# fab-jul/L3C-PyTorch

Hardware: AMD Instinct MI355X
Metric: MPix/s encode (net+CDF+AC) on 768x512 RGB (higher is better)
Workload: dtype f32; 1 GPU; L3C 0306_0001 (cr.cf, synthetic seeded checkpoint), batch of 768x512 synthetic RGB per GPU: net forward + fused logistic-mixture CDF head + HIP range coder -> bytes in HBM; checkpoint=calibrated, batch_per_gpu=128, image=768x512, coder_cus=0

## Files before the change

l3c-pytorch_amd/_lib.py:

```python
import ctypes
import os

import torch

_HERE = os.path.dirname(os.path.abspath(__file__))
LIB_PATH = os.environ.get('L3C_LIB') or os.path.join(_HERE, 'csrc', 'libl3c_hip.so')

c_i64, c_int, c_vp, c_f32 = ctypes.c_int64, ctypes.c_int, ctypes.c_void_p, ctypes.c_float


class L3CError(RuntimeError):
    pass


class ConvDesc(ctypes.Structure):
    _fields_ = [('inp', c_vp), ('in_cstride', c_int), ('in_coff', c_int),
                ('packed_w', c_vp), ('bias', c_vp),
                ('residual', c_vp), ('res_cstride', c_int), ('res_coff', c_int),
                ('out', c_vp), ('out_cstride', c_int), ('out_coff', c_int),
                ('B', c_int), ('Hin', c_int), ('Win', c_int), ('Cin', c_int), ('Cout', c_int),
                ('KS', c_int), ('stride', c_int), ('dilation', c_int), ('epilogue', c_int)]


class AcGroup(ctypes.Structure):
# ... 195 lines not shown
XCHECK_PROTOTYPES = {
    'l3c_conv_wino_packed_words': (c_i64, [c_int, c_int]),
    'l3c_conv_wino_pack_weights': (c_int, [c_vp, c_int, c_int, c_vp, c_vp]),
    'l3c_conv_wino': (c_int, [ctypes.POINTER(ConvDesc), c_vp]),
    'l3c_conv_wino_set_tiles_per_block': (c_int, [c_int]),
    'l3c_xcheck_sigmoid_exhaustive': (c_int, [c_vp, c_vp, c_vp]),
    'l3c_conv_wino4w_packed_words': (c_i64, [c_int, c_int]),
    'l3c_conv_wino4w_pack_weights': (c_int, [c_vp, c_int, c_int, c_vp, c_vp]),
    'l3c_conv_wino4w': (c_int, [ctypes.POINTER(ConvDesc), c_int, c_vp]),
}
XCHECK_SMALL_PROTOTYPES = {
    'l3c_xcheck_rgb_head': (c_int, [c_vp, c_vp, c_vp, c_vp, c_vp, c_vp, c_vp, c_int, c_int, c_int, c_int, c_vp, c_vp, c_vp]),
    'l3c_xcheck_to_q_quantize': (c_int, [c_vp, c_vp, c_vp, c_vp, c_i64, c_i64, c_int, c_int, c_int, c_vp, c_vp, c_vp, c_vp]),
    'l3c_xcheck_dec_head': (c_int, [c_vp, c_vp, c_vp, c_vp, c_i64, c_i64, c_int, c_int, c_vp, c_vp]),
}
XCHECK_LIB_PATH = os.environ.get('L3C_XCHECK_LIB') or os.path.join(_HERE, 'csrc', 'libl3c_hip_xcheck.so')

_lib = None
_xcheck = None


def load():
    global _lib
    if _lib is None:
        _snapshot_queues()
        if not os.path.isfile(LIB_PATH):
            raise L3CError('libl3c_hip.so not found at {} -- build it with `python l3c-pytorch_amd/csrc/build.py` '
                           '(or __graft_entry__.build()); there is no CPU fallback.'.format(LIB_PATH))
        lib = ctypes.CDLL(LIB_PATH)
        for name, (res, args) in PROTOTYPES.items():
            fn = getattr(lib, name)
            fn.restype, fn.argtypes = res, args
        if lib.l3c_abi_version() != ABI_VERSION:
            raise L3CError('ABI version mismatch: library {} != binding {}'.format(lib.l3c_abi_version(), ABI_VERSION))
        _lib = lib
    return _lib


def load_xcheck():
    global _xcheck
    if _xcheck is None:
        if not os.path.isfile(XCHECK_LIB_PATH):
            raise L3CError('libl3c_hip_xcheck.so not found at {} -- build it with `python l3c-pytorch_amd/csrc/build.py`'.format(XCHECK_LIB_PATH))
        lib = ctypes.CDLL(XCHECK_LIB_PATH)
        lib.l3c_last_error.restype = ctypes.c_char_p
        for name, (res, args) in list(XCHECK_PROTOTYPES.items()) + list(XCHECK_SMALL_PROTOTYPES.items()):
            fn = getattr(lib, name)
            fn.restype, fn.argtypes = res, args
        _xcheck = lib
    return _xcheck


def call_xcheck(name, *args):
    rc = getattr(load_xcheck(), name)(*args)
    if rc != 0:
        raise L3CError('libl3c_hip_xcheck: {} (status {})'.format(load_xcheck().l3c_last_error().decode(), rc))


def check(rc):
    if rc != 0:
        raise L3CError('libl3c_hip: {} (status {})'.format(load().l3c_last_error().decode(), rc))
# ... 60 lines not shown
```

l3c-pytorch_amd/csrc/ac_kernels.hip:

```cpp
#include <vector>

#include "ac_core.h"
#include "dmll_core.h"
#include "l3c_common.h"

namespace {

constexpr int kChunk = 64;

__device__ __forceinline__ int64_t iv_index(int64_t chunk, int64_t n_streams, int64_t s, int role, int j) {
    return ((chunk * n_streams + s) * 2 + role) * kChunk + j;
}

__global__ __launch_bounds__(256) void intervals_from_table_kernel(const uint16_t *__restrict__ cdf, int64_t row_stride,
                                                                   int Lp, const int16_t *__restrict__ sym,
                                                                   int64_t n_streams, int64_t n_sym,
                                                                   uint32_t *__restrict__ iv) {
    const int64_t n_chunks = (n_sym + kChunk - 1) / kChunk;
    const int64_t total = n_chunks * n_streams * kChunk;
    for (int64_t i = (int64_t)blockIdx.x * blockDim.x + threadIdx.x; i < total; i += (int64_t)gridDim.x * blockDim.x) {
        const int j = (int)(i % kChunk);
        const int64_t s = (i / kChunk) % n_streams;
        const int64_t chunk = i / kChunk / n_streams;
        const int64_t t = chunk * kChunk + j;
// ... 661 lines not shown

__device__ __forceinline__ Regs<4> window_full_row(const WindowCtx &w, int64_t b, int64_t n, int lane) {
    const int C = w.C, K = w.K, c = w.c;
    const float *px = w.P + (b * w.HW + n) * (int64_t)(4 * C * K);
    auto get = [&](int ch) { return px[ch]; };
    float x0 = 0.f, x1 = 0.f;
    if (c > 0) {
        x0 = (float)w.sym[(b * C + 0) * w.HW + n];
        if (c > 1) x1 = (float)w.sym[(b * C + 1) * w.HW + n];
    }
    const l3c::MixStats st = l3c::mix_stats(get, C, K, c);
    const float t0 = w.targets[lane], t1 = w.targets[lane + 64], t2 = w.targets[lane + 128], t3 = w.targets[lane + 192];
    float a0 = 0.0f, a1 = 0.0f, a2 = 0.0f, a3 = 0.0f;
    for (int k = 0; k < K; ++k) {
        const l3c::MixComponent m = l3c::mix_component(get, st, C, K, 1, c, k, x0, x1);
        const float inv = expf(-m.log_sigma);
        a0 = a0 + l3c::cdf_term(m.pi, m.mu, inv, t0);
        a1 = a1 + l3c::cdf_term(m.pi, m.mu, inv, t1);
        a2 = a2 + l3c::cdf_term(m.pi, m.mu, inv, t2);
        a3 = a3 + l3c::cdf_term(m.pi, m.mu, inv, t3);
    }
    const float scale = (float)(65536 - 256);
    return Regs<4>{l3c::cdf_quantise(a0, scale, lane), l3c::cdf_quantise(a1, scale, lane + 64), l3c::cdf_quantise(a2, scale, lane + 128),
                   l3c::cdf_quantise(a3, scale, lane + 192)};
}

__device__ __forceinline__ bool full_row_monotone(const Regs<4> &r, int lane) {
    const uint32_t na = (uint32_t)__shfl_down((int)r.a, 1, 64), nb = (uint32_t)__shfl_down((int)r.b, 1, 64);
    const uint32_t nc = (uint32_t)__shfl_down((int)r.c, 1, 64), nd = (uint32_t)__shfl_down((int)r.d, 1, 64);
    bool bad = lane < 63 && (!(r.a < na) || !(r.b < nb) || !(r.c < nc) || !(r.d < nd));
    const uint32_t b0 = lane_read(r.b, 0), c0 = lane_read(r.c, 0), d0 = lane_read(r.d, 0);
// ... 290 lines not shown
    }
}
struct LaneMixture {
    float pi, mu, inv;
};
__device__ __forceinline__ LaneMixture window_lane_mixture(const WindowCtx &w, int64_t b, int64_t n, int lane) {
    const int C = w.C, K = w.K, c = w.c;
    const float *px = w.P + (b * w.HW + n) * (int64_t)(4 * C * K);
    auto get = [&](int ch) { return px[ch]; };
    float x0 = 0.f, x1 = 0.f;
    if (c > 0) {
        x0 = (float)w.sym[(b * C + 0) * w.HW + n];
        if (c > 1) x1 = (float)w.sym[(b * C + 1) * w.HW + n];
    }
    const int k = lane < K ? lane : K - 1;
    l3c::MixStats st;
    st.max_logit = get(c * K);
    for (int j = 1; j < K; ++j) st.max_logit = fmaxf(st.max_logit, get(c * K + j));
    const float e_k = expf(get(c * K + k) - st.max_logit);
    st.denom = 0.0f;
    for (int j = 0; j < K; ++j) st.denom = st.denom + __builtin_bit_cast(float, __builtin_amdgcn_readlane(__builtin_bit_cast(int, e_k), j));
    const l3c::MixComponent m = l3c::mix_component_e(get, st, e_k, C, K, 1, c, k, x0, x1);
    return LaneMixture{m.pi, m.mu, expf(-m.log_sigma)};
}
__device__ __forceinline__ RowHi<1> window_row_at(const WindowCtx &w, const LaneMixture &mx, int wbase, int lane, bool &monotone) {
    const float t = w.targets[wbase + lane];
    float acc = 0.0f;
    for (int j = 0; j < w.K; ++j) {
        const float pi = __builtin_bit_cast(float, __builtin_amdgcn_readlane(__builtin_bit_cast(int, mx.pi), j));
        const float mu = __builtin_bit_cast(float, __builtin_amdgcn_readlane(__builtin_bit_cast(int, mx.mu), j));
        const float inv = __builtin_bit_cast(float, __builtin_amdgcn_readlane(__builtin_bit_cast(int, mx.inv), j));
        acc = acc + l3c::cdf_term(pi, mu, inv, t);
    }
    const uint32_t v = l3c::cdf_quantise(acc, (float)(65536 - 256), wbase + lane);
    const uint32_t nxt = (uint32_t)__shfl_down((int)v, 1, 64);
    monotone = !__any(lane < 63 && !(v < nxt));
    return RowHi<1>{v << 16};
}
// ... 815 lines not shown
```

l3c-pytorch_amd/csrc/build.py:

```python
import os
import subprocess
import sys

HERE = os.path.dirname(os.path.abspath(__file__))
SOURCES = ['l3c_api.hip', 'ac_kernels.hip', 'dmll_kernels.hip', 'conv_mfma.hip', 'conv_small.hip', 'container.hip', 'conv_pw.hip', 'conv_wino4.hip', 'decode_pipeline.hip',
           'net.hip', 'codec.hip']
XCHECK_SOURCES = ['l3c_api.hip', 'conv_wino.hip', 'xcheck_dmll.hip', 'conv_wino4w.hip', 'xcheck_small.hip']
HEADERS = ['ac_core.h', 'dmll_core.h', 'l3c_common.h', 'codec_plan.h', 'codec_plan_banded.h', os.path.join('..', '..', 'include', 'l3c_hip.h'), os.path.join('..', '..', 'include', 'l3c_xcheck.h'),
           os.path.join('..', '..', 'include', 'l3c_xcheck_small.h')]
LIB = os.path.join(HERE, 'libl3c_hip.so')
XCHECK_LIB = os.path.join(HERE, 'libl3c_hip_xcheck.so')
FLAGS = ['--offload-arch=gfx950', '-O3', '-std=c++17', '-fPIC', '-ffp-contract=off', '-Wall', '-Wno-unused-function']
SOURCE_FLAGS = {'conv_wino.hip': ['-fno-slp-vectorize'], 'conv_pw.hip': ['-fno-slp-vectorize'], 'conv_wino4.hip': ['-fno-slp-vectorize'],
                'conv_wino4w.hip': ['-fno-slp-vectorize']}


def _stale(target, deps):
    if not os.path.isfile(target):
        return True
    t = os.path.getmtime(target)
    return any(os.path.getmtime(d) > t for d in deps)


def build(force=False, verbose=False, extra=(), lib=LIB, objdir='_obj', xcheck=True):
# ... 47 lines not shown
```

l3c-pytorch_amd/csrc/dmll_core.h:

```cpp
#ifndef L3C_DMLL_CORE_H_
#define L3C_DMLL_CORE_H_

#include <hip/hip_runtime.h>

namespace l3c {

__device__ __forceinline__ float sigmoid_f(float a) { return 1.0f / (1.0f + expf(-a)); }

__device__ __forceinline__ float sigmoid_mid(float a) {
    const float kNegLog2e = __uint_as_float(0xbfb8aa3bu);
    const float kNegLog2eLo = __uint_as_float(0xb2a5705fu);
    const float t = kNegLog2e * a;
    const float n = __builtin_rintf(t);
    float f = t - n;
    float c = __builtin_fmaf(a, kNegLog2e, -t);
    c = __builtin_fmaf(kNegLog2eLo, a, c);
    f = f + c;
    const float e = __builtin_amdgcn_ldexpf(__builtin_amdgcn_exp2f(f), (int)n);
    const float d = 1.0f + e;
    float r = __builtin_amdgcn_rcpf(d);
    r = __builtin_fmaf(__builtin_fmaf(-d, r, 1.0f), r, r);
    float q = r;
    q = __builtin_fmaf(__builtin_fmaf(-d, q, 1.0f), r, q);
    return __builtin_fmaf(__builtin_fmaf(-d, q, 1.0f), r, q);
}

__device__ __forceinline__ float sigmoid_sat(float a) {
    if (a >= 16.7f) return 1.0f;
    if (a <= -89.0f) return 0.0f;
    if (a > -80.0f) return sigmoid_mid(a);
    return sigmoid_f(a);
}

constexpr float kLogScalesMin = -7.0f;

struct MixStats {
    float max_logit, denom;
};

template <class Get>
__device__ __forceinline__ MixStats mix_stats(Get get, int C, int K, int c) {
    MixStats s;
    s.max_logit = get(c * K);
    for (int k = 1; k < K; ++k) s.max_logit = fmaxf(s.max_logit, get(c * K + k));
    s.denom = 0.0f;
    for (int k = 0; k < K; ++k) s.denom = s.denom + expf(get(c * K + k) - s.max_logit);
    return s;
}

struct MixComponent {
    float pi, mu, log_sigma;
};

template <class Get>
__device__ __forceinline__ MixComponent mix_component_e(Get get, const MixStats &st, float e_k, int C, int K, int rgb, int c, int k,
                                                        float x0, float x1) {
    const int CK = C * K;
    MixComponent m;
    m.pi = e_k / st.denom;
    m.mu = get(CK + c * K + k);
    m.log_sigma = fmaxf(get(2 * CK + c * K + k), kLogScalesMin);
    if (rgb && c == 1) {
        m.mu = m.mu + sigmoid_f(get(3 * CK + k)) * x0;
    } else if (rgb && c == 2) {
        const float a = sigmoid_f(get(3 * CK + K + k)) * x0;
        const float b = sigmoid_f(get(3 * CK + 2 * K + k)) * x1;
        m.mu = m.mu + (a + b);
    }
    return m;
}

template <class Get>
__device__ __forceinline__ MixComponent mix_component(Get get, const MixStats &st, int C, int K, int rgb, int c, int k,
                                                      float x0, float x1) {
    return mix_component_e(get, st, expf(get(c * K + k) - st.max_logit), C, K, rgb, c, k, x0, x1);
}

__device__ __forceinline__ float cdf_term(float pi, float mu, float inv_sigma, float target) {
    return pi * sigmoid_sat((target - mu) * inv_sigma);
}

__device__ __forceinline__ uint32_t cdf_quantise(float cdf, float scale, int l) {
    return (uint32_t)((int)rintf(cdf * scale) + l) & 0xFFFFu;
}

constexpr int kWinLp = 65;
constexpr int kWinTop = 63;
constexpr int kWinMaxOffset = 192;

constexpr int kWinBad = 0x40000000;
// ... 23 lines not shown
```

l3c-pytorch_amd/csrc/dmll_kernels.hip:

```cpp
#include "ac_core.h"
#include "dmll_core.h"
#include "l3c_common.h"

namespace {

using l3c::sigmoid_f;
using l3c::sigmoid_sat;
using l3c::kLogScalesMin;
using l3c::MixStats;
using l3c::MixComponent;
using l3c::mix_stats;
using l3c::mix_component;
using l3c::mix_component_e;
using l3c::cdf_term;
using l3c::cdf_quantise;

struct TileDiv {
    unsigned q4, magic;
};
static TileDiv tile_div(int Kp, int max_pix) {
    TileDiv d{0u, 0u};
#ifdef L3C_IV_SCALAR_FILL
    return d;
#endif
// ... 85 lines not shown
__global__ __launch_bounds__(256) void cdf_table_kernel(const float *__restrict__ targets, const float *__restrict__ pi,
                                                        const float *__restrict__ mu, const float *__restrict__ ls,
                                                        int64_t HW, int K, int Lp, uint16_t *__restrict__ cdf) {
    __shared__ float s_pi[kTablePix][kMaxK], s_mu[kTablePix][kMaxK], s_inv[kTablePix][kMaxK];
    __shared__ float s_t[260];
    const int64_t img = blockIdx.y;
    const int64_t pix0 = (int64_t)blockIdx.x * kTablePix;
    const int npix = (int)((HW - pix0) < kTablePix ? (HW - pix0) : kTablePix);
    const int tid = threadIdx.x;
    for (int i = tid; i < kTablePix * K; i += 256) {
        const int p = i % kTablePix, k = i / kTablePix;
        if (p < npix) {
            const int64_t o = (img * K + k) * HW + pix0 + p;
            s_pi[p][k] = pi[o];
            s_mu[p][k] = mu[o];
            s_inv[p][k] = expf(-ls[o]);
        }
    }
    for (int i = tid; i < Lp; i += 256) s_t[i] = targets[i];
    __syncthreads();
    const float scale = (float)(65536 - (Lp - 1));
    const int count = npix * Lp;
    uint16_t *out = cdf + (img * HW + pix0) * Lp;
    const bool aligned4 = ((reinterpret_cast<uintptr_t>(out) & 3) == 0);
    for (int e = tid * 2; e < count; e += 512) {
        uint32_t v[2];
#pragma unroll
        for (int h = 0; h < 2; ++h) {
            const int ee = e + h < count ? e + h : e;
            const int p = ee / Lp, l = ee - p * Lp;
            const float t = s_t[l];
// ... 49 lines not shown
    if (off >= range_len) return;
    const int64_t pix0 = range0 + off;
    const int npix = (int)((range_len - off) < kTablePix ? (range_len - off) : kTablePix);
    const int tid = threadIdx.x;
    const bool window = win_stats && l3c::use_window(win_stats[b]);
    const float *src = P + pix0 * Kp;
    fill_tile<256>(tile, src, npix, Kp, ld, dv, tid);
    for (int i = tid; i < Lp; i += 256) s_t[i] = targets[i];
    __syncthreads();
    for (int i = tid; i < kTablePix * K; i += 256) {
        const int p = i % kTablePix, k = i / kTablePix;
        if (p < npix) {
            const float *px = tile + p * ld;
            float mx = px[c * K];
            for (int j = 1; j < K; ++j) mx = fmaxf(mx, px[c * K + j]);
            s_e[p][k] = expf(px[c * K + k] - mx);
            if (k == 0) s_max[p] = mx;
        }
    }
    __syncthreads();
    for (int i = tid; i < kTablePix * K; i += 256) {
        const int p = i % kTablePix, k = i / kTablePix;
        if (p < npix) {
            const float *px = tile + p * ld;
            const int64_t n = pix0 + p;
            float x0 = 0.f, x1 = 0.f;
            if (rgb && c > 0) {
                x0 = (float)sym[0 * HW + n];
                if (c > 1) x1 = (float)sym[1 * HW + n];
            }
            MixStats st;
            st.max_logit = s_max[p];
            st.denom = 0.0f;
            for (int j = 0; j < K; ++j) st.denom = st.denom + s_e[p][j];
            const MixComponent m = mix_component_e([&](int ch) { return px[ch]; }, st, s_e[p][k], C, K, rgb, c, k, x0, x1);
            s_pi[p][k] = m.pi;
            s_mu[p][k] = m.mu;
            s_inv[p][k] = expf(-m.log_sigma);
        }
    }
    __syncthreads();
    const float scale = (float)(65536 - (Lp - 1));
    auto pixel_w0 = [&](int p) {
        float mean = 0.0f;
        for (int k = 0; k < K; ++k) mean = mean + s_pi[p][k] * s_mu[p][k];
        return l3c::window_offset(mean);
    };
    const int lane = tid & 63;
    if (window) {
        const int p = tid >> 3, q = tid & 7;
        bool bad = false;
        if (p < npix) {
            const int w0 = pixel_w0(p);
// ... 64 lines not shown
    }
    if (not_monotone) {
        __syncthreads();
        const int runs = (count + 127) >> 7;
        for (int j = tid; j + 1 < runs; j += 256) {
            const int m = (128 * j + 127) % Lp;
            bad = bad || (m <= Lp - 3 && !(s_edge[j][1] < s_edge[j + 1][0]));
        }
        if (__any(bad) && lane == 0) atomicOr(not_monotone, 1);
    }
}


constexpr int kHeadPix = 64;

template <int NT>
__global__ __launch_bounds__(NT) void encode_intervals_kernel(const float *__restrict__ P, const int16_t *__restrict__ sym,
                                                               const float *__restrict__ targets, int64_t HW, int C, int K,
                                                               int rgb, int Lp, uint32_t *__restrict__ iv, TileDiv dv) {
    extern __shared__ __attribute__((aligned(16))) float tile[];
    const int Kp = (rgb ? 4 : 3) * C * K;
    const int ld = Kp + 1;
    const int64_t b = blockIdx.y;
    const int64_t chunk = blockIdx.x;
    const int64_t pix0 = chunk * kHeadPix;
    const int npix = (int)((HW - pix0) < kHeadPix ? (HW - pix0) : kHeadPix);
    const int tid = threadIdx.x;
    const float *src = P + (b * HW + pix0) * Kp;
    constexpr int nthreads = NT;
    fill_tile<NT>(tile, src, npix, Kp, ld, dv, tid);
    __syncthreads();
    const float scale = (float)(65536 - (Lp - 1));
    const int64_t n_streams = (int64_t)gridDim.y * C;
    for (int w = tid; w < kHeadPix * C; w += nthreads) {
        const int p = w % kHeadPix, c = w / kHeadPix;
        uint32_t word0 = 0, word1 = 0;
        if (p < npix) {
            const float *px = tile + p * ld;
            auto get = [&](int ch) { return px[ch]; };
            const int64_t n = pix0 + p;
            const int x = sym[(b * C + c) * HW + n];
            float x0 = 0.f, x1 = 0.f;
            if (rgb && c > 0) {
                x0 = (float)sym[(b * C + 0) * HW + n];
                if (c > 1) x1 = (float)sym[(b * C + 1) * HW + n];
            }
            const float t_lo = targets[x];
            const float t_hi = targets[x + 1];
            MixStats st;
            st.max_logit = get(c * K);
            for (int k = 1; k < K; ++k) st.max_logit = fmaxf(st.max_logit, get(c * K + k));
            float e[kMaxK];
            st.denom = 0.0f;
#pragma unroll
            for (int k = 0; k < kMaxK; ++k) {
                e[k] = k < K ? expf(get(c * K + k) - st.max_logit) : 0.0f;
                if (k < K) st.denom = st.denom + e[k];
            }
            float acc_lo = 0.0f, acc_hi = 0.0f;
#pragma unroll
            for (int k = 0; k < kMaxK; ++k) {
                if (k >= K) break;
                const MixComponent m = mix_component_e(get, st, e[k], C, K, rgb, c, k, x0, x1);
                const float inv = expf(-m.log_sigma);
                acc_lo = acc_lo + cdf_term(m.pi, m.mu, inv, t_lo);
                acc_hi = acc_hi + cdf_term(m.pi, m.mu, inv, t_hi);
            }
            const uint32_t c_lo = cdf_quantise(acc_lo, scale, x);
            const uint32_t c_hi = (x == Lp - 2) ? 0x10000u : cdf_quantise(acc_hi, scale, x + 1);
            word0 = l3c::role_word(c_lo, c_hi, 0);
            word1 = l3c::role_word(c_lo, c_hi, 1);
        }
        uint32_t *dst = iv + (chunk * n_streams + b * C + c) * (2 * kHeadPix) + p;
        dst[0] = word0;
        dst[kHeadPix] = word1;
    }
}


__device__ __forceinline__ float softplus_f(float x) { return x > 20.0f ? x : log1pf(expf(x)); }

__global__ __launch_bounds__(256) void nll_kernel(const float *__restrict__ P, const float *__restrict__ xs, int64_t HW,
                                                  int C, int K, int rgb, float x_lower, float x_upper, float half_bin,
                                                  float *__restrict__ nll) {
    extern __shared__ __attribute__((aligned(16))) float tile[];
    const int Kp = (rgb ? 4 : 3) * C * K;
    const int CK = C * K;
    const int ld = Kp + 1;
    const int64_t b = blockIdx.y;
    const int64_t pix0 = (int64_t)blockIdx.x * kHeadPix;
    const int npix = (int)((HW - pix0) < kHeadPix ? (HW - pix0) : kHeadPix);
// ... 253 lines not shown
                              int K, int rgb, int Lp, uint32_t *intervals, l3c_stream_t stream) {
    L3C_REQUIRE(P && sym && targets && intervals, "null pointer");
    L3C_REQUIRE(B > 0 && B < 65536 && HW > 0 && C > 0 && K > 0, "bad shape");
    L3C_REQUIRE(K <= kMaxK, "K out of range");
    L3C_REQUIRE(!rgb || C == 3, "lambda coupling is only defined for C == 3");
    L3C_REQUIRE(Lp >= 2 && Lp <= 65536, "Lp out of range");
    const int Kp = (rgb ? 4 : 3) * C * K;
    const size_t lds = (size_t)kHeadPix * (Kp + 1) * sizeof(float);
    L3C_REQUIRE(lds <= 64 * 1024, "Kp too large for the LDS tile");
    const dim3 grid((unsigned)((HW + kHeadPix - 1) / kHeadPix), (unsigned)B);
#ifdef L3C_IV_THREADS_256
    const int nthreads = 256;
#else
    const int nthreads = kHeadPix * C == 320 ? 320 : 256;
#endif
    if (nthreads == 320)
        hipLaunchKernelGGL(encode_intervals_kernel<320>, grid, dim3(320), lds, l3c::as_stream(stream), P, sym, targets, HW, C, K, rgb, Lp,
                           intervals, tile_div(Kp, kHeadPix));
    else
        hipLaunchKernelGGL(encode_intervals_kernel<256>, grid, dim3(256), lds, l3c::as_stream(stream), P, sym, targets, HW, C, K, rgb, Lp,
                           intervals, tile_div(Kp, kHeadPix));
    return l3c::check_launch("encode_intervals_kernel");
}

int l3c_dmll_nll(const float *P, const float *x, int64_t B, int64_t HW, int C, int K, int rgb, float x_min, float x_max,
                 int L, float *nll, l3c_stream_t stream) {
    L3C_REQUIRE(P && x && nll, "null pointer");
    L3C_REQUIRE(B > 0 && B < 65536 && HW > 0 && C > 0, "bad shape");
    L3C_REQUIRE(K > 0 && K <= kMaxK, "K out of range (1..16)");
    L3C_REQUIRE(!rgb || C == 3, "lambda coupling is only defined for C == 3");
// ... 48 lines not shown
```

l3c-pytorch_amd/csrc/xcheck_dmll.hip:

```cpp
#include "../../include/l3c_xcheck.h"
#include "dmll_core.h"
#include "l3c_common.h"

namespace {

__global__ __launch_bounds__(256) void sigmoid_exhaustive_kernel(unsigned long long *mismatches, uint32_t *first_bad) {
    const uint64_t stride = (uint64_t)gridDim.x * blockDim.x;
    unsigned long long bad = 0;
    for (uint64_t i = (uint64_t)blockIdx.x * blockDim.x + threadIdx.x; i < (1ull << 32); i += stride) {
        const uint32_t bits = (uint32_t)i;
        const float a = __uint_as_float(bits);
        const float want = l3c::sigmoid_f(a), got = l3c::sigmoid_sat(a);
        const bool same = __float_as_uint(want) == __float_as_uint(got) || (want != want && got != got);
        if (!same) {
            ++bad;
            atomicMin(first_bad, bits);
        }
    }
    if (bad) atomicAdd(mismatches, bad);
}

}

extern "C" int l3c_xcheck_sigmoid_exhaustive(unsigned long long *mismatches_dev, uint32_t *first_bad_dev, l3c_stream_t stream) {
    L3C_REQUIRE(mismatches_dev && first_bad_dev, "null pointer");
    hipLaunchKernelGGL(sigmoid_exhaustive_kernel, dim3(4096), dim3(256), 0, l3c::as_stream(stream), mismatches_dev, first_bad_dev);
    return l3c::check_launch("sigmoid_exhaustive_kernel");
}
```

Measured before the change: 187.6 MPix/s.

## Replace libm exp/div in mixture CDF head with range-guarded fast paths and specialised kernels

Introduces exp_lean/exp_reduced, a fast exponential built on exp2 with hi/lo log2e reduction and a libm fallback outside a safe range. It also replaces the softmax division with a refined reciprocal whenever the denominator and numerator lie in safe ranges, and swaps sigmoid_f for sigmoid_sat in the coupling terms. The encode-intervals kernel gains compile-time C/K-specialised item evaluation, using wave-uniform __all checks to choose fast paths and a noinline per-lane fallback. A frozen copy of the old kernel and exhaustive exp/division cross-check kernels are added to verify bit-exactness. The aim is to cut transcendental and division cost in the CDF head, at the price of extra branches, more code and register pressure.

```diff
diff --git a/include/l3c_xcheck_dmll.h b/include/l3c_xcheck_dmll.h
--- /dev/null
+++ b/include/l3c_xcheck_dmll.h
@@ -0,0 +1,22 @@
+#ifndef L3C_XCHECK_DMLL_H_
+#define L3C_XCHECK_DMLL_H_
+
+#include "l3c_hip.h"
+
+#ifdef __cplusplus
+extern "C" {
+#endif
+
+int l3c_xcheck_encode_intervals(const float *P, const int16_t *sym, const float *targets, int64_t B, int64_t HW, int C, int K, int rgb,
+                                int Lp, uint32_t *intervals, l3c_stream_t stream);
+
+int l3c_xcheck_exp_exhaustive(unsigned long long *mismatches_dev, uint32_t *first_bad_dev, l3c_stream_t stream);
+
+int l3c_xcheck_softmax_div(const float *divisors_dev, int n_divisors, uint64_t n_random, uint64_t seed,
+                           unsigned long long *mismatches_dev, unsigned long long *first_bad_dev, l3c_stream_t stream);
+
+#ifdef __cplusplus
+}
+#endif
+
+#endif
diff --git a/l3c-pytorch_amd/_lib.py b/l3c-pytorch_amd/_lib.py
--- a/l3c-pytorch_amd/_lib.py
+++ b/l3c-pytorch_amd/_lib.py
@@ -233,6 +233,11 @@
     'l3c_xcheck_to_q_quantize': (c_int, [c_vp, c_vp, c_vp, c_vp, c_i64, c_i64, c_int, c_int, c_int, c_vp, c_vp, c_vp, c_vp]),
     'l3c_xcheck_dec_head': (c_int, [c_vp, c_vp, c_vp, c_vp, c_i64, c_i64, c_int, c_int, c_vp, c_vp]),
 }
+XCHECK_DMLL_PROTOTYPES = {
+    'l3c_xcheck_encode_intervals': (c_int, [c_vp, c_vp, c_vp, c_i64, c_i64, c_int, c_int, c_int, c_int, c_vp, c_vp]),
+    'l3c_xcheck_exp_exhaustive': (c_int, [c_vp, c_vp, c_vp]),
+    'l3c_xcheck_softmax_div': (c_int, [c_vp, c_int, ctypes.c_uint64, ctypes.c_uint64, c_vp, c_vp, c_vp]),
+}
 XCHECK_LIB_PATH = os.environ.get('L3C_XCHECK_LIB') or os.path.join(_HERE, 'csrc', 'libl3c_hip_xcheck.so')
 
 _lib = None
@@ -263,7 +268,7 @@
             raise L3CError('libl3c_hip_xcheck.so not found at {} -- build it with `python l3c-pytorch_amd/csrc/build.py`'.format(XCHECK_LIB_PATH))
         lib = ctypes.CDLL(XCHECK_LIB_PATH)
         lib.l3c_last_error.restype = ctypes.c_char_p
-        for name, (res, args) in list(XCHECK_PROTOTYPES.items()) + list(XCHECK_SMALL_PROTOTYPES.items()):
+        for name, (res, args) in list(XCHECK_PROTOTYPES.items()) + list(XCHECK_SMALL_PROTOTYPES.items()) + list(XCHECK_DMLL_PROTOTYPES.items()):
             fn = getattr(lib, name)
             fn.restype, fn.argtypes = res, args
         _xcheck = lib
diff --git a/l3c-pytorch_amd/csrc/ac_kernels.hip b/l3c-pytorch_amd/csrc/ac_kernels.hip
--- a/l3c-pytorch_amd/csrc/ac_kernels.hip
+++ b/l3c-pytorch_amd/csrc/ac_kernels.hip
@@ -699,7 +699,7 @@
     float a0 = 0.0f, a1 = 0.0f, a2 = 0.0f, a3 = 0.0f;
     for (int k = 0; k < K; ++k) {
         const l3c::MixComponent m = l3c::mix_component(get, st, C, K, 1, c, k, x0, x1);
-        const float inv = expf(-m.log_sigma);
+        const float inv = l3c::exp_lean(-m.log_sigma);
         a0 = a0 + l3c::cdf_term(m.pi, m.mu, inv, t0);
         a1 = a1 + l3c::cdf_term(m.pi, m.mu, inv, t1);
         a2 = a2 + l3c::cdf_term(m.pi, m.mu, inv, t2);
@@ -1020,14 +1020,14 @@
         if (c > 1) x1 = (float)w.sym[(b * C + 1) * w.HW + n];
     }
     const int k = lane < K ? lane : K - 1;
-    l3c::MixStats st;
-    st.max_logit = get(c * K);
-    for (int j = 1; j < K; ++j) st.max_logit = fmaxf(st.max_logit, get(c * K + j));
-    const float e_k = expf(get(c * K + k) - st.max_logit);
-    st.denom = 0.0f;
-    for (int j = 0; j < K; ++j) st.denom = st.denom + __builtin_bit_cast(float, __builtin_amdgcn_readlane(__builtin_bit_cast(int, e_k), j));
+    float max_logit = get(c * K);
+    for (int j = 1; j < K; ++j) max_logit = fmaxf(max_logit, get(c * K + j));
+    const float e_k = l3c::exp_lean(get(c * K + k) - max_logit);
+    float denom = 0.0f;
+    for (int j = 0; j < K; ++j) denom = denom + __builtin_bit_cast(float, __builtin_amdgcn_readlane(__builtin_bit_cast(int, e_k), j));
+    const l3c::MixStats st = l3c::mix_stats_of(max_logit, denom);
     const l3c::MixComponent m = l3c::mix_component_e(get, st, e_k, C, K, 1, c, k, x0, x1);
-    return LaneMixture{m.pi, m.mu, expf(-m.log_sigma)};
+    return LaneMixture{m.pi, m.mu, l3c::exp_lean(-m.log_sigma)};
 }
 __device__ __forceinline__ RowHi<1> window_row_at(const WindowCtx &w, const LaneMixture &mx, int wbase, int lane, bool &monotone) {
     const float t = w.targets[wbase + lane];
diff --git a/l3c-pytorch_amd/csrc/build.py b/l3c-pytorch_amd/csrc/build.py
--- a/l3c-pytorch_amd/csrc/build.py
+++ b/l3c-pytorch_amd/csrc/build.py
@@ -7,7 +7,7 @@
            'net.hip', 'codec.hip']
 XCHECK_SOURCES = ['l3c_api.hip', 'conv_wino.hip', 'xcheck_dmll.hip', 'conv_wino4w.hip', 'xcheck_small.hip']
 HEADERS = ['ac_core.h', 'dmll_core.h', 'l3c_common.h', 'codec_plan.h', 'codec_plan_banded.h', os.path.join('..', '..', 'include', 'l3c_hip.h'), os.path.join('..', '..', 'include', 'l3c_xcheck.h'),
-           os.path.join('..', '..', 'include', 'l3c_xcheck_small.h')]
+           os.path.join('..', '..', 'include', 'l3c_xcheck_small.h'), os.path.join('..', '..', 'include', 'l3c_xcheck_dmll.h')]
 LIB = os.path.join(HERE, 'libl3c_hip.so')
 XCHECK_LIB = os.path.join(HERE, 'libl3c_hip_xcheck.so')
 FLAGS = ['--offload-arch=gfx950', '-O3', '-std=c++17', '-fPIC', '-ffp-contract=off', '-Wall', '-Wno-unused-function']
diff --git a/l3c-pytorch_amd/csrc/dmll_core.h b/l3c-pytorch_amd/csrc/dmll_core.h
--- a/l3c-pytorch_amd/csrc/dmll_core.h
+++ b/l3c-pytorch_amd/csrc/dmll_core.h
@@ -7,16 +7,24 @@
 
 __device__ __forceinline__ float sigmoid_f(float a) { return 1.0f / (1.0f + expf(-a)); }
 
-__device__ __forceinline__ float sigmoid_mid(float a) {
-    const float kNegLog2e = __uint_as_float(0xbfb8aa3bu);
-    const float kNegLog2eLo = __uint_as_float(0xb2a5705fu);
-    const float t = kNegLog2e * a;
+__device__ __forceinline__ float exp_reduced(float x) {
+    const float kLog2e = __uint_as_float(0x3fb8aa3bu);
+    const float kLog2eLo = __uint_as_float(0x32a5705fu);
+    const float t = x * kLog2e;
     const float n = __builtin_rintf(t);
     float f = t - n;
-    float c = __builtin_fmaf(a, kNegLog2e, -t);
-    c = __builtin_fmaf(kNegLog2eLo, a, c);
+    float c = __builtin_fmaf(x, kLog2e, -t);
+    c = __builtin_fmaf(x, kLog2eLo, c);
     f = f + c;
-    const float e = __builtin_amdgcn_ldexpf(__builtin_amdgcn_exp2f(f), (int)n);
+    return __builtin_amdgcn_ldexpf(__builtin_amdgcn_exp2f(f), (int)n);
+}
+__device__ __forceinline__ float exp_lean(float x) {
+    if (x > -100.0f && x < 88.0f) return exp_reduced(x);
+    return expf(x);
+}
+
+__device__ __forceinline__ float sigmoid_mid(float a) {
+    const float e = exp_reduced(-a);
     const float d = 1.0f + e;
     float r = __builtin_amdgcn_rcpf(d);
     r = __builtin_fmaf(__builtin_fmaf(-d, r, 1.0f), r, r);
@@ -36,16 +44,34 @@
 
 struct MixStats {
     float max_logit, denom;
+    float rcp_denom, e_min;
 };
+__device__ __forceinline__ MixStats mix_stats_of(float max_logit, float denom) {
+    MixStats s;
+    s.max_logit = max_logit;
+    s.denom = denom;
+    const float r = __builtin_amdgcn_rcpf(denom);
+    s.rcp_denom = __builtin_fmaf(__builtin_fmaf(-denom, r, 1.0f), r, r);
+    s.e_min = (denom >= 1.0f && denom <= 16.0f) ? __uint_as_float(0x0d800000u) : __builtin_inff();
+    return s;
+}
+__device__ __forceinline__ float softmax_div_lean(float e, float d, float r) {
+    float q = e * r;
+    q = __builtin_fmaf(__builtin_fmaf(-d, q, e), r, q);
+    return __builtin_fmaf(__builtin_fmaf(-d, q, e), r, q);
+}
+__device__ __forceinline__ float softmax_div(float e, const MixStats &st) {
+    if (e >= st.e_min) return softmax_div_lean(e, st.denom, st.rcp_denom);
+    return e / st.denom;
+}
 
 template <class Get>
 __device__ __forceinline__ MixStats mix_stats(Get get, int C, int K, int c) {
-    MixStats s;
-    s.max_logit = get(c * K);
-    for (int k = 1; k < K; ++k) s.max_logit = fmaxf(s.max_logit, get(c * K + k));
-    s.denom = 0.0f;
-    for (int k = 0; k < K; ++k) s.denom = s.denom + expf(get(c * K + k) - s.max_logit);
-    return s;
+    float max_logit = get(c * K);
+    for (int k = 1; k < K; ++k) max_logit = fmaxf(max_logit, get(c * K + k));
+    float denom = 0.0f;
+    for (int k = 0; k < K; ++k) denom = denom + exp_lean(get(c * K + k) - max_logit);
+    return mix_stats_of(max_logit, denom);
 }
 
 struct MixComponent {
@@ -57,14 +83,14 @@
                                                         float x0, float x1) {
     const int CK = C * K;
     MixComponent m;
-    m.pi = e_k / st.denom;
+    m.pi = softmax_div(e_k, st);
     m.mu = get(CK + c * K + k);
     m.log_sigma = fmaxf(get(2 * CK + c * K + k), kLogScalesMin);
     if (rgb && c == 1) {
-        m.mu = m.mu + sigmoid_f(get(3 * CK + k)) * x0;
+        m.mu = m.mu + sigmoid_sat(get(3 * CK + k)) * x0;
     } else if (rgb && c == 2) {
-        const float a = sigmoid_f(get(3 * CK + K + k)) * x0;
-        const float b = sigmoid_f(get(3 * CK + 2 * K + k)) * x1;
+        const float a = sigmoid_sat(get(3 * CK + K + k)) * x0;
+        const float b = sigmoid_sat(get(3 * CK + 2 * K + k)) * x1;
         m.mu = m.mu + (a + b);
     }
     return m;
@@ -73,7 +99,7 @@
 template <class Get>
 __device__ __forceinline__ MixComponent mix_component(Get get, const MixStats &st, int C, int K, int rgb, int c, int k,
                                                       float x0, float x1) {
-    return mix_component_e(get, st, expf(get(c * K + k) - st.max_logit), C, K, rgb, c, k, x0, x1);
+    return mix_component_e(get, st, exp_lean(get(c * K + k) - st.max_logit), C, K, rgb, c, k, x0, x1);
 }
 
 __device__ __forceinline__ float cdf_term(float pi, float mu, float inv_sigma, float target) {
diff --git a/l3c-pytorch_amd/csrc/dmll_kernels.hip b/l3c-pytorch_amd/csrc/dmll_kernels.hip
--- a/l3c-pytorch_amd/csrc/dmll_kernels.hip
+++ b/l3c-pytorch_amd/csrc/dmll_kernels.hip
@@ -6,6 +6,10 @@
 
 using l3c::sigmoid_f;
 using l3c::sigmoid_sat;
+using l3c::sigmoid_mid;
+using l3c::exp_lean;
+using l3c::mix_stats_of;
+using l3c::softmax_div_lean;
 using l3c::kLogScalesMin;
 using l3c::MixStats;
 using l3c::MixComponent;
@@ -123,7 +127,7 @@
             const int64_t o = (img * K + k) * HW + pix0 + p;
             s_pi[p][k] = pi[o];
             s_mu[p][k] = mu[o];
-            s_inv[p][k] = expf(-ls[o]);
+            s_inv[p][k] = exp_lean(-ls[o]);
         }
     }
     for (int i = tid; i < Lp; i += 256) s_t[i] = targets[i];
@@ -203,7 +207,7 @@
             const float *px = tile + p * ld;
             float mx = px[c * K];
             for (int j = 1; j < K; ++j) mx = fmaxf(mx, px[c * K + j]);
-            s_e[p][k] = expf(px[c * K + k] - mx);
+            s_e[p][k] = exp_lean(px[c * K + k] - mx);
             if (k == 0) s_max[p] = mx;
         }
     }
@@ -218,14 +222,13 @@
                 x0 = (float)sym[0 * HW + n];
                 if (c > 1) x1 = (float)sym[1 * HW + n];
             }
-            MixStats st;
-            st.max_logit = s_max[p];
-            st.denom = 0.0f;
-            for (int j = 0; j < K; ++j) st.denom = st.denom + s_e[p][j];
+            float denom = 0.0f;
+            for (int j = 0; j < K; ++j) denom = denom + s_e[p][j];
+            const MixStats st = mix_stats_of(s_max[p], denom);
             const MixComponent m = mix_component_e([&](int ch) { return px[ch]; }, st, s_e[p][k], C, K, rgb, c, k, x0, x1);
             s_pi[p][k] = m.pi;
             s_mu[p][k] = m.mu;
-            s_inv[p][k] = expf(-m.log_sigma);
+            s_inv[p][k] = exp_lean(-m.log_sigma);
         }
     }
     __syncthreads();
@@ -320,6 +323,31 @@
 
 constexpr int kHeadPix = 64;
 
+__device__ __forceinline__ void interval_item_runtime(const float *px, int C, int K, int rgb, int c, float x0, float x1, float t_lo, float t_hi,
+                                                      float &acc_lo, float &acc_hi) {
+    auto get = [&](int ch) { return px[ch]; };
+    float max_logit = get(c * K);
+    for (int k = 1; k < K; ++k) max_logit = fmaxf(max_logit, get(c * K + k));
+    float e[kMaxK];
+    float denom = 0.0f;
+#pragma unroll
+    for (int k = 0; k < kMaxK; ++k) {
+        e[k] = k < K ? exp_lean(get(c * K + k) - max_logit) : 0.0f;
+        if (k < K) denom = denom + e[k];
+    }
+    const MixStats st = mix_stats_of(max_logit, denom);
+    acc_lo = 0.0f;
+    acc_hi = 0.0f;
+#pragma unroll
+    for (int k = 0; k < kMaxK; ++k) {
+        if (k >= K) break;
+        const MixComponent m = mix_component_e(get, st, e[k], C, K, rgb, c, k, x0, x1);
+        const float inv = exp_lean(-m.log_sigma);
+        acc_lo = acc_lo + cdf_term(m.pi, m.mu, inv, t_lo);
+        acc_hi = acc_hi + cdf_term(m.pi, m.mu, inv, t_hi);
+    }
+}
+
 template <int NT>
 __global__ __launch_bounds__(NT) void encode_intervals_kernel(const float *__restrict__ P, const int16_t *__restrict__ sym,
                                                                const float *__restrict__ targets, int64_t HW, int C, int K,
@@ -343,7 +371,6 @@
         uint32_t word0 = 0, word1 = 0;
         if (p < npix) {
             const float *px = tile + p * ld;
-            auto get = [&](int ch) { return px[ch]; };
             const int64_t n = pix0 + p;
             const int x = sym[(b * C + c) * HW + n];
             float x0 = 0.f, x1 = 0.f;
@@ -351,27 +378,8 @@
                 x0 = (float)sym[(b * C + 0) * HW + n];
                 if (c > 1) x1 = (float)sym[(b * C + 1) * HW + n];
             }
-            const float t_lo = targets[x];
-            const float t_hi = targets[x + 1];
-            MixStats st;
-            st.max_logit = get(c * K);
-            for (int k = 1; k < K; ++k) st.max_logit = fmaxf(st.max_logit, get(c * K + k));
-            float e[kMaxK];
-            st.denom = 0.0f;
-#pragma unroll
-            for (int k = 0; k < kMaxK; ++k) {
-                e[k] = k < K ? expf(get(c * K + k) - st.max_logit) : 0.0f;
-                if (k < K) st.denom = st.denom + e[k];
-            }
-            float acc_lo = 0.0f, acc_hi = 0.0f;
-#pragma unroll
-            for (int k = 0; k < kMaxK; ++k) {
-                if (k >= K) break;
-                const MixComponent m = mix_component_e(get, st, e[k], C, K, rgb, c, k, x0, x1);
-                const float inv = expf(-m.log_sigma);
-                acc_lo = acc_lo + cdf_term(m.pi, m.mu, inv, t_lo);
-                acc_hi = acc_hi + cdf_term(m.pi, m.mu, inv, t_hi);
-            }
+            float acc_lo, acc_hi;
+            interval_item_runtime(px, C, K, rgb, c, x0, x1, targets[x], targets[x + 1], acc_lo, acc_hi);
             const uint32_t c_lo = cdf_quantise(acc_lo, scale, x);
             const uint32_t c_hi = (x == Lp - 2) ? 0x10000u : cdf_quantise(acc_hi, scale, x + 1);
             word0 = l3c::role_word(c_lo, c_hi, 0);
@@ -381,6 +389,150 @@
         dst[0] = word0;
         dst[kHeadPix] = word1;
     }
+}
+
+__device__ __attribute__((noinline)) float2 sigmoid_sat_pair(float a, float b) { return make_float2(sigmoid_sat(a), sigmoid_sat(b)); }
+
+__device__ __forceinline__ void sigmoid_pair(float a, float b, float &sa, float &sb) {
+    if (__all(a > -80.0f && b < 16.7f)) {
+        sa = sigmoid_mid(a);
+        sb = sigmoid_mid(b);
+    } else {
+        const float2 s = sigmoid_sat_pair(a, b);
+        sa = s.x;
+        sb = s.y;
+    }
+}
+
+__device__ __attribute__((noinline)) float2 interval_item_per_lane(const float *px, int C, int K, int rgb, int c, float x0, float x1, float t_lo,
+                                                                   float t_hi) {
+    float2 acc;
+    interval_item_runtime(px, C, K, rgb, c, x0, x1, t_lo, t_hi, acc.x, acc.y);
+    return acc;
+}
+
+template <int COUPLE, int C, int K>
+__device__ __forceinline__ void interval_item(const float *__restrict__ px, int c, float x0, float x1, float t_lo, float t_hi, float &acc_lo,
+                                              float &acc_hi) {
+    constexpr int CK = C * K;
+    const float *__restrict__ pc = px + c * K;
+    float logit[K], log_sigma[K];
+#pragma unroll
+    for (int k = 0; k < K; ++k) {
+        logit[k] = pc[k];
+        log_sigma[k] = fmaxf(pc[2 * CK + k], kLogScalesMin);
+    }
+    float max_logit = logit[0], min_logit = logit[0], max_log_sigma = log_sigma[0];
+#pragma unroll
+    for (int k = 1; k < K; ++k) {
+        max_logit = fmaxf(max_logit, logit[k]);
+        min_logit = fminf(min_logit, logit[k]);
+        max_log_sigma = fmaxf(max_log_sigma, log_sigma[k]);
+    }
+    if (!__all(min_logit - max_logit > -100.0f && max_log_sigma < 100.0f)) {
+        const float2 acc = interval_item_per_lane(px, C, K, COUPLE != 0, c, x0, x1, t_lo, t_hi);
+        acc_lo = acc.x;
+        acc_hi = acc.y;
+        return;
+    }
+    float e[K];
+    float denom = 0.0f;
+#pragma unroll
+    for (int k = 0; k < K; ++k) {
+        e[k] = l3c::exp_reduced(logit[k] - max_logit);
+        denom = denom + e[k];
+    }
+    const MixStats st = mix_stats_of(max_logit, denom);
+    acc_lo = 0.0f;
+    acc_hi = 0.0f;
+#pragma unroll
+    for (int k = 0; k < K; ++k) {
+        float pi;
+        if (__all(e[k] >= st.e_min)) {
+            pi = softmax_div_lean(e[k], st.denom, st.rcp_denom);
+        } else {
+            pi = e[k] / st.denom;
+        }
+        float mu = pc[CK + k];
+        if (COUPLE == 1) {
+            const float la = px[3 * CK + k];
+            float sa;
+            if (__all(la > -80.0f && la < 16.7f)) {
+                sa = sigmoid_mid(la);
+            } else {
+                sa = sigmoid_sat_pair(la, la).x;
+            }
+            mu = mu + sa * x0;
+        } else if (COUPLE == 2) {
+            const float la = px[3 * CK + K + k], lb = px[3 * CK + 2 * K + k];
+            float sa, sb;
+            if (__all(la > -80.0f && la < 16.7f && lb > -80.0f && lb < 16.7f)) {
+                sa = sigmoid_mid(la);
+                sb = sigmoid_mid(lb);
+            } else {
+                const float2 s = sigmoid_sat_pair(la, lb);
+                sa = s.x;
+                sb = s.y;
+            }
+            mu = mu + (sa * x0 + sb * x1);
+        }
+        const float inv = l3c::exp_reduced(-log_sigma[k]);
+        float s_lo, s_hi;
+        sigmoid_pair((t_lo - mu) * inv, (t_hi - mu) * inv, s_lo, s_hi);
+        acc_lo = acc_lo + pi * s_lo;
+        acc_hi = acc_hi + pi * s_hi;
+    }
+}
+
+template <int NT, bool RGB, int C, int K>
+__global__ __launch_bounds__(NT) void encode_intervals_kernel_lean(const float *__restrict__ P, const int16_t *__restrict__ sym,
+                                                                    const float *__restrict__ targets, int64_t HW, int Lp,
+                                                                    uint32_t *__restrict__ iv, TileDiv dv) {
+    extern __shared__ __attribute__((aligned(16))) float tile[];
+    static_assert(kHeadPix == 64 && NT % 64 == 0 && NT >= kHeadPix * C, "one (pixel, channel) item per thread, one channel per wavefront");
+    static_assert(!RGB || C == 3, "lambda coupling is only defined for C == 3");
+    constexpr int Kp = (RGB ? 4 : 3) * C * K;
+    constexpr int ld = Kp + 1;
+    const int64_t b = blockIdx.y;
+    const int64_t chunk = blockIdx.x;
+    const int64_t pix0 = chunk * kHeadPix;
+    const int npix = (int)((HW - pix0) < kHeadPix ? (HW - pix0) : kHeadPix);
+    const int tid = threadIdx.x;
+    fill_tile<NT>(tile, P + (b * HW + pix0) * Kp, npix, Kp, ld, dv, tid);
+    __syncthreads();
+    const int p = tid & (kHeadPix - 1);
+    const int c = __builtin_amdgcn_readfirstlane(tid >> 6);
+    if (c >= C) return;
+    const float scale = (float)(65536 - (Lp - 1));
+    const int64_t n_streams = (int64_t)gridDim.y * C;
+    uint32_t word0 = 0, word1 = 0;
+    if (p < npix) {
+        const float *px = tile + p * ld;
+        const int64_t n = pix0 + p;
+        const int x = sym[(b * C + c) * HW + n];
+        float x0 = 0.f, x1 = 0.f;
+        if (RGB && c > 0) {
+            x0 = (float)sym[(b * C + 0) * HW + n];
+            if (c > 1) x1 = (float)sym[(b * C + 1) * HW + n];
+        }
+        const float t_lo = targets[x];
+        const float t_hi = targets[x + 1];
+        float acc_lo, acc_hi;
+        if (RGB && c == 1) {
+            interval_item<1, C, K>(px, c, x0, x1, t_lo, t_hi, acc_lo, acc_hi);
+        } else if (RGB && c == 2) {
+            interval_item<2, C, K>(px, c, x0, x1, t_lo, t_hi, acc_lo, acc_hi);
+        } else {
+            interval_item<0, C, K>(px, c, x0, x1, t_lo, t_hi, acc_lo, acc_hi);
+        }
+        const uint32_t c_lo = cdf_quantise(acc_lo, scale, x);
+        const uint32_t c_hi = (x == Lp - 2) ? 0x10000u : cdf_quantise(acc_hi, scale, x + 1);
+        word0 = l3c::role_word(c_lo, c_hi, 0);
+        word1 = l3c::role_word(c_lo, c_hi, 1);
+    }
+    uint32_t *dst = iv + (chunk * n_streams + b * C + c) * (2 * kHeadPix) + p;
+    dst[0] = word0;
+    dst[kHeadPix] = word1;
 }
 
 
@@ -664,6 +816,18 @@
 #else
     const int nthreads = kHeadPix * C == 320 ? 320 : 256;
 #endif
+#ifndef L3C_IV_GENERIC
+    if (rgb && C == 3 && K == 10) {
+        hipLaunchKernelGGL((encode_intervals_kernel_lean<256, true, 3, 10>), grid, dim3(256), lds, l3c::as_stream(stream), P, sym, targets, HW,
+                           Lp, intervals, tile_div(Kp, kHeadPix));
+        return l3c::check_launch("encode_intervals_kernel_lean");
+    }
+    if (!rgb && C == 5 && K == 10) {
+        hipLaunchKernelGGL((encode_intervals_kernel_lean<320, false, 5, 10>), grid, dim3(320), lds, l3c::as_stream(stream), P, sym, targets, HW,
+                           Lp, intervals, tile_div(Kp, kHeadPix));
+        return l3c::check_launch("encode_intervals_kernel_lean");
+    }
+#endif
     if (nthreads == 320)
         hipLaunchKernelGGL(encode_intervals_kernel<320>, grid, dim3(320), lds, l3c::as_stream(stream), P, sym, targets, HW, C, K, rgb, Lp,
                            intervals, tile_div(Kp, kHeadPix));
diff --git a/l3c-pytorch_amd/csrc/xcheck_dmll.hip b/l3c-pytorch_amd/csrc/xcheck_dmll.hip
--- a/l3c-pytorch_amd/csrc/xcheck_dmll.hip
+++ b/l3c-pytorch_amd/csrc/xcheck_dmll.hip
@@ -1,4 +1,6 @@
 #include "../../include/l3c_xcheck.h"
+#include "../../include/l3c_xcheck_dmll.h"
+#include "ac_core.h"
 #include "dmll_core.h"
 #include "l3c_common.h"
 
@@ -20,6 +22,261 @@
     if (bad) atomicAdd(mismatches, bad);
 }
 
+__global__ __launch_bounds__(256) void exp_exhaustive_kernel(unsigned long long *mismatches, uint32_t *first_bad) {
+    const uint64_t stride = (uint64_t)gridDim.x * blockDim.x;
+    unsigned long long bad = 0;
+    for (uint64_t i = (uint64_t)blockIdx.x * blockDim.x + threadIdx.x; i < (1ull << 32); i += stride) {
+        const uint32_t bits = (uint32_t)i;
+        const float a = __uint_as_float(bits);
+        const float want = expf(a), got = l3c::exp_lean(a);
+        const bool same = __float_as_uint(want) == __float_as_uint(got) || (want != want && got != got);
+        if (!same) {
+            ++bad;
+            atomicMin(first_bad, bits);
+        }
+    }
+    if (bad) atomicAdd(mismatches, bad);
+}
+
+__device__ __forceinline__ void softmax_div_check(float e, const l3c::MixStats &st, unsigned long long &bad, unsigned long long *first_bad) {
+    const float want = e / st.denom, got = l3c::softmax_div(e, st);
+    const bool same = __float_as_uint(want) == __float_as_uint(got) || (want != want && got != got);
+    if (!same) {
+        ++bad;
+        atomicMin(first_bad, ((unsigned long long)__float_as_uint(e) << 32) | __float_as_uint(st.denom));
+    }
+}
+
+constexpr uint32_t kOneBits = 0x3f800000u;
+
+__global__ __launch_bounds__(256) void softmax_div_all_kernel(const float *__restrict__ divisors, unsigned long long *mismatches,
+                                                              unsigned long long *first_bad) {
+    const l3c::MixStats st = l3c::mix_stats_of(0.0f, divisors[blockIdx.y]);
+    const uint32_t stride = gridDim.x * blockDim.x;
+    unsigned long long bad = 0;
+    for (uint64_t i = (uint64_t)blockIdx.x * blockDim.x + threadIdx.x; i <= kOneBits; i += stride)
+        softmax_div_check(__uint_as_float((uint32_t)i), st, bad, first_bad);
+    if (bad) atomicAdd(mismatches, bad);
+}
+
+__device__ __forceinline__ uint64_t splitmix64(uint64_t z) {
+    z += 0x9e3779b97f4a7c15ull;
+    z = (z ^ (z >> 30)) * 0xbf58476d1ce4e5b9ull;
+    z = (z ^ (z >> 27)) * 0x94d049bb133111ebull;
+    return z ^ (z >> 31);
+}
+
+__global__ __launch_bounds__(256) void softmax_div_random_kernel(uint64_t n, uint64_t seed, unsigned long long *mismatches,
+                                                                 unsigned long long *first_bad) {
+    const uint64_t stride = (uint64_t)gridDim.x * blockDim.x;
+    unsigned long long bad = 0;
+    for (uint64_t i = (uint64_t)blockIdx.x * blockDim.x + threadIdx.x; i < n; i += stride) {
+        const uint64_t r = splitmix64(seed + i);
+        const uint32_t eb = (uint32_t)(((r & 0xffffffffull) * (kOneBits + 1ull)) >> 32);
+        const uint32_t db = kOneBits + (uint32_t)(((r >> 32) * (0x41800000ull - kOneBits + 1ull)) >> 32);
+        softmax_div_check(__uint_as_float(eb), l3c::mix_stats_of(0.0f, __uint_as_float(db)), bad, first_bad);
+    }
+    if (bad) atomicAdd(mismatches, bad);
+}
+
+namespace frozen {
+
+__device__ __forceinline__ float sigmoid_f(float a) { return 1.0f / (1.0f + expf(-a)); }
+
+__device__ __forceinline__ float sigmoid_mid(float a) {
+    const float kNegLog2e = __uint_as_float(0xbfb8aa3bu);
+    const float kNegLog2eLo = __uint_as_float(0xb2a5705fu);
+    const float t = kNegLog2e * a;
+    const float n = __builtin_rintf(t);
+    float f = t - n;
+    float c = __builtin_fmaf(a, kNegLog2e, -t);
+    c = __builtin_fmaf(kNegLog2eLo, a, c);
+    f = f + c;
+    const float e = __builtin_amdgcn_ldexpf(__builtin_amdgcn_exp2f(f), (int)n);
+    const float d = 1.0f + e;
+    float r = __builtin_amdgcn_rcpf(d);
+    r = __builtin_fmaf(__builtin_fmaf(-d, r, 1.0f), r, r);
+    float q = r;
+    q = __builtin_fmaf(__builtin_fmaf(-d, q, 1.0f), r, q);
+    return __builtin_fmaf(__builtin_fmaf(-d, q, 1.0f), r, q);
+}
+
+__device__ __forceinline__ float sigmoid_sat(float a) {
+    if (a >= 16.7f) return 1.0f;
+    if (a <= -89.0f) return 0.0f;
+    if (a > -80.0f) return sigmoid_mid(a);
+    return sigmoid_f(a);
+}
+
+constexpr float kLogScalesMin = -7.0f;
+
+struct MixStats {
+    float max_logit, denom;
+};
+
+struct MixComponent {
+    float pi, mu, log_sigma;
+};
+
+template <class Get>
+__device__ __forceinline__ MixComponent mix_component_e(Get get, const MixStats &st, float e_k, int C, int K, int rgb, int c, int k,
+                                                        float x0, float x1) {
+    const int CK = C * K;
+    MixComponent m;
+    m.pi = e_k / st.denom;
+    m.mu = get(CK + c * K + k);
+    m.log_sigma = fmaxf(get(2 * CK + c * K + k), kLogScalesMin);
+    if (rgb && c == 1) {
+        m.mu = m.mu + sigmoid_f(get(3 * CK + k)) * x0;
+    } else if (rgb && c == 2) {
+        const float a = sigmoid_f(get(3 * CK + K + k)) * x0;
+        const float b = sigmoid_f(get(3 * CK + 2 * K + k)) * x1;
+        m.mu = m.mu + (a + b);
+    }
+    return m;
+}
+
+__device__ __forceinline__ float cdf_term(float pi, float mu, float inv_sigma, float target) {
+    return pi * sigmoid_sat((target - mu) * inv_sigma);
+}
+
+__device__ __forceinline__ uint32_t cdf_quantise(float cdf, float scale, int l) {
+    return (uint32_t)((int)rintf(cdf * scale) + l) & 0xFFFFu;
+}
+
+
+struct TileDiv {
+    unsigned q4, magic;
+};
+static TileDiv tile_div(int Kp, int max_pix) {
+    TileDiv d{0u, 0u};
+#ifdef L3C_IV_SCALAR_FILL
+    return d;
+#endif
+    if (Kp % 4 != 0) return d;
+    const unsigned q = (unsigned)(Kp / 4);
+    const unsigned magic = ((1u << 20) + q - 1u) / q;
+    for (unsigned i = 0; i < (unsigned)max_pix * q; ++i)
+        if (i / q != (unsigned)(((unsigned long long)i * magic) >> 20)) return d;
+    d.q4 = q;
+    d.magic = magic;
+    return d;
+}
+template <int NT>
+__device__ __forceinline__ void fill_tile(float *__restrict__ tile, const float *__restrict__ src, int npix, int Kp, int ld, TileDiv dv, int tid) {
+    if (dv.q4 && (reinterpret_cast<uintptr_t>(src) & 15) == 0) {
+        constexpr int U = 4;
+        const float4 *src4 = reinterpret_cast<const float4 *>(src);
+        const int n4 = npix * (int)dv.q4;
+        for (int i0 = tid; i0 < n4; i0 += NT * U) {
+            float4 v[U];
+#pragma unroll
+            for (int u = 0; u < U; ++u) {
+                const int i = i0 + u * NT;
+                v[u] = src4[i < n4 ? i : i0];
+            }
+#pragma unroll
+            for (int u = 0; u < U; ++u) {
+                const int i = i0 + u * NT;
+                if (i < n4) {
+                    const int p = (int)(((unsigned)i * dv.magic) >> 20);
+                    float *dst = tile + p * ld + (i - p * (int)dv.q4) * 4;
+                    dst[0] = v[u].x;
+                    dst[1] = v[u].y;
+                    dst[2] = v[u].z;
+                    dst[3] = v[u].w;
+                }
+            }
+        }
+    } else {
+        constexpr int U = 8;
+        const int n = npix * Kp;
+        for (int i0 = tid; i0 < n; i0 += NT * U) {
+            float v[U];
+#pragma unroll
+            for (int u = 0; u < U; ++u) {
+                const int i = i0 + u * NT;
+                v[u] = src[i < n ? i : i0];
+            }
+#pragma unroll
+            for (int u = 0; u < U; ++u) {
+                const int i = i0 + u * NT;
+                if (i < n) tile[(i / Kp) * ld + (i % Kp)] = v[u];
+            }
+        }
+    }
+}
+
+constexpr int kMaxK = 16;
+
+
+constexpr int kHeadPix = 64;
+
+template <int NT>
+__global__ __launch_bounds__(NT) void encode_intervals_kernel(const float *__restrict__ P, const int16_t *__restrict__ sym,
+                                                               const float *__restrict__ targets, int64_t HW, int C, int K,
+                                                               int rgb, int Lp, uint32_t *__restrict__ iv, TileDiv dv) {
+    extern __shared__ __attribute__((aligned(16))) float tile[];
+    const int Kp = (rgb ? 4 : 3) * C * K;
+    const int ld = Kp + 1;
+    const int64_t b = blockIdx.y;
+    const int64_t chunk = blockIdx.x;
+    const int64_t pix0 = chunk * kHeadPix;
+    const int npix = (int)((HW - pix0) < kHeadPix ? (HW - pix0) : kHeadPix);
+    const int tid = threadIdx.x;
+    const float *src = P + (b * HW + pix0) * Kp;
+    constexpr int nthreads = NT;
+    fill_tile<NT>(tile, src, npix, Kp, ld, dv, tid);
+    __syncthreads();
+    const float scale = (float)(65536 - (Lp - 1));
+    const int64_t n_streams = (int64_t)gridDim.y * C;
+    for (int w = tid; w < kHeadPix * C; w += nthreads) {
+        const int p = w % kHeadPix, c = w / kHeadPix;
+        uint32_t word0 = 0, word1 = 0;
+        if (p < npix) {
+            const float *px = tile + p * ld;
+            auto get = [&](int ch) { return px[ch]; };
+            const int64_t n = pix0 + p;
+            const int x = sym[(b * C + c) * HW + n];
+            float x0 = 0.f, x1 = 0.f;
+            if (rgb && c > 0) {
+                x0 = (float)sym[(b * C + 0) * HW + n];
+                if (c > 1) x1 = (float)sym[(b * C + 1) * HW + n];
+            }
+            const float t_lo = targets[x];
+            const float t_hi = targets[x + 1];
+            MixStats st;
+            st.max_logit = get(c * K);
+            for (int k = 1; k < K; ++k) st.max_logit = fmaxf(st.max_logit, get(c * K + k));
+            float e[kMaxK];
+            st.denom = 0.0f;
+#pragma unroll
+            for (int k = 0; k < kMaxK; ++k) {
+                e[k] = k < K ? expf(get(c * K + k) - st.max_logit) : 0.0f;
+                if (k < K) st.denom = st.denom + e[k];
+            }
+            float acc_lo = 0.0f, acc_hi = 0.0f;
+#pragma unroll
+            for (int k = 0; k < kMaxK; ++k) {
+                if (k >= K) break;
+                const MixComponent m = mix_component_e(get, st, e[k], C, K, rgb, c, k, x0, x1);
+                const float inv = expf(-m.log_sigma);
+                acc_lo = acc_lo + cdf_term(m.pi, m.mu, inv, t_lo);
+                acc_hi = acc_hi + cdf_term(m.pi, m.mu, inv, t_hi);
+            }
+            const uint32_t c_lo = cdf_quantise(acc_lo, scale, x);
+            const uint32_t c_hi = (x == Lp - 2) ? 0x10000u : cdf_quantise(acc_hi, scale, x + 1);
+            word0 = l3c::role_word(c_lo, c_hi, 0);
+            word1 = l3c::role_word(c_lo, c_hi, 1);
+        }
+        uint32_t *dst = iv + (chunk * n_streams + b * C + c) * (2 * kHeadPix) + p;
+        dst[0] = word0;
+        dst[kHeadPix] = word1;
+    }
+}
+
+}
+
 }
 
 extern "C" int l3c_xcheck_sigmoid_exhaustive(unsigned long long *mismatches_dev, uint32_t *first_bad_dev, l3c_stream_t stream) {
@@ -27,3 +284,56 @@
     hipLaunchKernelGGL(sigmoid_exhaustive_kernel, dim3(4096), dim3(256), 0, l3c::as_stream(stream), mismatches_dev, first_bad_dev);
     return l3c::check_launch("sigmoid_exhaustive_kernel");
 }
+
+extern "C" int l3c_xcheck_exp_exhaustive(unsigned long long *mismatches_dev, uint32_t *first_bad_dev, l3c_stream_t stream) {
+    L3C_REQUIRE(mismatches_dev && first_bad_dev, "null pointer");
+    hipLaunchKernelGGL(exp_exhaustive_kernel, dim3(4096), dim3(256), 0, l3c::as_stream(stream), mismatches_dev, first_bad_dev);
+    return l3c::check_launch("exp_exhaustive_kernel");
+}
+
+extern "C" int l3c_xcheck_softmax_div(const float *divisors_dev, int n_divisors, uint64_t n_random, uint64_t seed,
+                                      unsigned long long *mismatches_dev, unsigned long long *first_bad_dev, l3c_stream_t stream) {
+    L3C_REQUIRE(mismatches_dev && first_bad_dev, "null pointer");
+    L3C_REQUIRE(n_divisors >= 0 && n_divisors <= 65535 && (n_divisors == 0 || divisors_dev), "0..65535 divisors");
+    if (n_divisors > 0) {
+        hipLaunchKernelGGL(softmax_div_all_kernel, dim3(1024, (unsigned)n_divisors), dim3(256), 0, l3c::as_stream(stream), divisors_dev,
+                           mismatches_dev, first_bad_dev);
+        const int rc = l3c::check_launch("softmax_div_all_kernel");
+        if (rc != L3C_OK) return rc;
+    }
+    if (n_random > 0) {
+        hipLaunchKernelGGL(softmax_div_random_kernel, dim3(4096), dim3(256), 0, l3c::as_stream(stream), n_random, seed, mismatches_dev,
+                           first_bad_dev);
+        return l3c::check_launch("softmax_div_random_kernel");
+    }
+    return L3C_OK;
+}
+
+extern "C" {
+using namespace frozen;
+int l3c_xcheck_encode_intervals(const float *P, const int16_t *sym, const float *targets, int64_t B, int64_t HW, int C,
+                              int K, int rgb, int Lp, uint32_t *intervals, l3c_stream_t stream) {
+    L3C_REQUIRE(P && sym && targets && intervals, "null pointer");
+    L3C_REQUIRE(B > 0 && B < 65536 && HW > 0 && C > 0 && K > 0, "bad shape");
+    L3C_REQUIRE(K <= kMaxK, "K out of range");
+    L3C_REQUIRE(!rgb || C == 3, "lambda coupling is only defined for C == 3");
+    L3C_REQUIRE(Lp >= 2 && Lp <= 65536, "Lp out of range");
+    const int Kp = (rgb ? 4 : 3) * C * K;
+    const size_t lds = (size_t)kHeadPix * (Kp + 1) * sizeof(float);
+    L3C_REQUIRE(lds <= 64 * 1024, "Kp too large for the LDS tile");
+    const dim3 grid((unsigned)((HW + kHeadPix - 1) / kHeadPix), (unsigned)B);
+#ifdef L3C_IV_THREADS_256
+    const int nthreads = 256;
+#else
+    const int nthreads = kHeadPix * C == 320 ? 320 : 256;
+#endif
+    if (nthreads == 320)
+        hipLaunchKernelGGL(encode_intervals_kernel<320>, grid, dim3(320), lds, l3c::as_stream(stream), P, sym, targets, HW, C, K, rgb, Lp,
+                           intervals, tile_div(Kp, kHeadPix));
+    else
+        hipLaunchKernelGGL(encode_intervals_kernel<256>, grid, dim3(256), lds, l3c::as_stream(stream), P, sym, targets, HW, C, K, rgb, Lp,
+                           intervals, tile_div(Kp, kHeadPix));
+    return l3c::check_launch("encode_intervals_kernel");
+}
+
+}
```

Measured after the change: 189.4 MPix/s (median of 6 runs). Within noise of the previous version (+1.0%).
